# ZhuoyangLiu2005/MLA

Measured on AMD Instinct MI355X. Metric: training samples/sec + step-time, MLA-Llama2-7B bf16, higher is better.
Workload: dtype bf16; 1 GPU; BASELINE.json configs[1]: MLA-Llama2-7B SFT, use_pointcloud+use_contrastive, 672x672(+mask) image + 1024 points + 32 text tokens, per-GPU batch 8 x 4 diffusion repeats = 32 x 548 tokens; model=mla-llama2-7b, global_batch=8, seq_len=548, parallelism=single-gpu, activation_save_level=1, optimizer=fused AdamW + grad clip inside the timed region

## Files before the change

### include/mla_hip.h

```cpp
#ifndef MLA_HIP_H
#define MLA_HIP_H

#include <stddef.h>
#include <stdint.h>

#ifdef __cplusplus
extern "C" {
#endif

typedef struct ihipStream_t* mla_stream_t;

const char* mla_last_error(void);
int mla_query(int what);
const char* mla_gemm_source_id(void);
int mla_selftest(const void* src_1k, int* out_tr_256, void* out_glds_1k, mla_stream_t stream);
int mla_calib_mfma(const void* operands, float* out, int blocks, int iters, double* flops_per_launch, mla_stream_t stream);
int mla_dispatch_probe(int* out, int blocks, int hold_us, mla_stream_t stream);

int mla_gemm_bf16(const void* A, const void* B, void* C, const void* R, const void* bias, int M, int N, int K, int lda, int ldb,
                  int ldc, int ldr, int a_mode, int b_mode, int out_fp32, int accumulate, float alpha, int force_generic,
                  mla_stream_t stream);
int mla_gemm_bf16_ws(const void* A, const void* B, void* C, const void* R, const void* bias, int M, int N, int K, int lda, int ldb,
                     int ldc, int ldr, int a_mode, int b_mode, int out_fp32, int accumulate, float alpha, int force_generic,
                     float* workspace, size_t workspace_bytes, mla_stream_t stream);
// ... 42 lines not shown
int mla_act_fwd(const void* x, void* y, long long n, int kind, mla_stream_t stream);
int mla_act_bwd(const void* dy, const void* x, void* dx, long long n, int kind, mla_stream_t stream);

int mla_cast_f32_to_bf16(const float* x, void* y, long long n, mla_stream_t stream);
int mla_cast_bf16_to_f32(const void* x, float* y, long long n, mla_stream_t stream);
int mla_add_bf16(const void* a, const void* b, void* y, long long n, mla_stream_t stream);
int mla_gather_rows_bf16(const void* src, const long long* idx, void* out, long long rows, int H, int scatter, mla_stream_t stream);

int mla_transpose_bf16(const void* src, void* dst, long long R, int C, long long ld, long long ldt, mla_stream_t stream);
int mla_rmsnorm_apply_t(const void* x, const void* w, const float* rstd, void* dst, long long rows, int H, long long ldt,
                        mla_stream_t stream);
int mla_swiglu_fwd_t(const void* gu, void* dst, long long rows, int I, long long ldt, mla_stream_t stream);
int mla_swiglu_fwd_dual(const void* gu, void* act, void* actT, long long rows, int I, long long ldt, mla_stream_t stream);
int mla_swiglu_bwd_t(const void* dact, const void* gu, void* dgu, void* dguT, long long rows, int I, long long ldt, mla_stream_t stream);

int mla_embedding_fwd(const long long* ids, const void* table, void* out, long long tokens, int H, int vocab, mla_stream_t stream);
int mla_embedding_bwd(const long long* ids, const void* dy, float* grad, float* workspace, long long tokens, int H, int vocab,
                      mla_stream_t stream);

int mla_adamw_step(float* p, const float* g, float* m, float* v, void* p16, long long n, float lr, float beta1, float beta2,
                   float eps, float weight_decay, int step, const float* grad_scale, mla_stream_t stream);
int mla_adamw_step_groups(float* p, const float* g, float* m, float* v, void* p16, long long n, long long n_decay, float lr, float beta1,
                          float beta2, float eps, float weight_decay, int step, const float* grad_scale, mla_stream_t stream);
int mla_sumsq_f32(const float* x, long long n, float* out, int accumulate, float* workspace, size_t workspace_bytes,
                  mla_stream_t stream);
int mla_sum_partials(const float* partial, int n, float* out, int accumulate, mla_stream_t stream);
int mla_clip_coef(const float* sumsq, float max_norm, float* coef, float* norm_out, mla_stream_t stream);

int mla_q_sample(const float* x0, const float* noise, const long long* t, const float* sqrt_ac, const float* sqrt_1mac, float* out,
                 int batch, int per, int nsteps, mla_stream_t stream);

int mla_attn_fwd(const void* q, const void* k, const void* v, void* o, float* lse, const int* seqlens, int B, int S, int H,
                 int head_dim, long long ld_qkv, long long ld_o, float scale, mla_stream_t stream);
int mla_attn_fwd_g(const void* q, const void* k, const void* v, void* o, float* lse, const int* seqlens, int B, int S, int H,
                   int head_dim, long long ld_qkv, long long ld_o, float scale, int grp_start, int grp_len, const int* grp_starts,
                   mla_stream_t stream);
int mla_attn_bwd_g(const void* q, const void* k, const void* v, const void* o, const void* dout, const float* lse, const int* seqlens,
                   void* dq, void* dk, void* dv, float* delta, int B, int S, int H, int head_dim, long long ld_qkv, long long ld_o,
                   float scale, const float* rope_cos, const float* rope_sin, void* dqT, void* dkT, void* dvT, void* oT,
                   long long ldt, int* head_sync, long long head_sync_ints, int grp_start, int grp_len, const int* grp_starts,
                   int rope_per_sample, mla_stream_t stream);
long long mla_attn_bwd_sync_ints(int B, int H);
int mla_attn_bwd(const void* q, const void* k, const void* v, const void* o, const void* dout, const float* lse, const int* seqlens,
                 void* dq, void* dk, void* dv, float* delta, int B, int S, int H, int head_dim, long long ld_qkv, long long ld_o,
                 float scale, const float* rope_cos, const float* rope_sin, int* head_sync, long long head_sync_ints,
                 mla_stream_t stream);
// ... 170 lines not shown
```

### mla_amd/csrc/elementwise.hip

```cpp
#include "common.h"
#include <math.h>

namespace {


constexpr int NORM_MAXC = 4;

__global__ __launch_bounds__(256) void rmsnorm_fwd_kernel(const bf16_t* __restrict__ x, const bf16_t* __restrict__ w,
                                                          bf16_t* __restrict__ y, float* __restrict__ rstd_out,
                                                          int rows, int H, float eps) {
  __shared__ float scratch[16];
  const int row = blockIdx.x;
  const int nchunk = H >> 3;
  const bf16_t* xr = x + (size_t)row * H;
  float xv[NORM_MAXC][8];
  float ss = 0.f;
#pragma unroll
  for (int c = 0; c < NORM_MAXC; ++c) {
    const int ch = threadIdx.x + c * 256;
    if (ch < nchunk) {
      const u32x4_t v = *(const u32x4_t*)(xr + ch * 8);
      unpack8(v, xv[c]);
#pragma unroll
      for (int j = 0; j < 8; ++j) ss += xv[c][j] * xv[c][j];
// ... 660 lines not shown
      if (i >= hi) continue;
      const float decay = i < n4_decay ? decay_on : 1.f;
#pragma unroll
      for (int r = 0; r < 4; ++r) {
        float pp = p4[u][r], mm = m4[u][r], vv = v4[u][r];
        adamw_elem(pp, g4[u][r], mm, vv, gs, decay, beta1, beta2, step, isq, eps);
        p4[u][r] = pp; m4[u][r] = mm; v4[u][r] = vv;
      }
      if (NT) {
        __builtin_nontemporal_store(p4[u], p + i); __builtin_nontemporal_store(m4[u], m + i); __builtin_nontemporal_store(v4[u], v + i);
      } else {
        p[i] = p4[u]; m[i] = m4[u]; v[i] = v4[u];
      }
      if (p16) {
        u32x2_t o;
        o[0] = pack2bf(p4[u][0], p4[u][1]);
        o[1] = pack2bf(p4[u][2], p4[u][3]);
        if (NT) __builtin_nontemporal_store(o, p16 + i); else p16[i] = o;
      }
    }
  }
}

__global__ __launch_bounds__(256) void sumsq_partial_kernel(const float* __restrict__ x, float* __restrict__ partial, long long n) {
  __shared__ float scratch[16];
  float s0 = 0.f, s1 = 0.f;
  const long long n4 = n >> 2;
  const f32x4_t* x4 = (const f32x4_t*)x;
  for (long long i = (long long)blockIdx.x * 256 + threadIdx.x; i < n4; i += (long long)gridDim.x * 256) {
    const f32x4_t v = x4[i];
    s0 += v[0] * v[0] + v[1] * v[1];
    s1 += v[2] * v[2] + v[3] * v[3];
  }
  if (blockIdx.x == 0 && threadIdx.x < (n & 3)) { const float v = x[(n4 << 2) + threadIdx.x]; s0 += v * v; }
  const float s = block_sum(s0 + s1, scratch);
  if (threadIdx.x == 0) partial[blockIdx.x] = s;
}
__global__ __launch_bounds__(256) void sum_final_kernel(const float* __restrict__ partial, float* __restrict__ out, int P,
                                                        int accumulate) {
  __shared__ float scratch[16];
  float s = 0.f;
  int i0 = 0;
  if ((((uintptr_t)partial) & 15) == 0) {
    const f32x4_t* p4 = (const f32x4_t*)partial;
    const int n4 = P >> 2;
    f32x4_t a0 = {0.f, 0.f, 0.f, 0.f}, a1 = a0, a2 = a0, a3 = a0;
// ... 240 lines not shown
    else if (variant == 3) ADAMW_LAUNCH(1, false);
    else if (variant == 4) ADAMW_LAUNCH(2, false);
    else ADAMW_LAUNCH(4, true);
#undef ADAMW_LAUNCH
  }
  const long long done = n4 * 4;
  if (done < n)
    hipLaunchKernelGGL(adamw_kernel, dim3(grid_for(n - done, 8192)), dim3(256), 0, stream, p + done, g + done, m + done, v + done,
                       p16 ? (bf16_t*)p16 + done : (bf16_t*)nullptr, n - done, lr, beta1, beta2, eps, weight_decay, bc1, bc2, grad_scale,
                       n_decay > done ? n_decay - done : 0);
  MLA_LAUNCH_CHECK();
}
extern "C" int mla_adamw_step(float* p, const float* g, float* m, float* v, void* p16, long long n, float lr, float beta1,
                              float beta2, float eps, float weight_decay, int step, const float* grad_scale,
                              hipStream_t stream) {
  return adamw_impl(p, g, m, v, p16, n, n, lr, beta1, beta2, eps, weight_decay, step, grad_scale, stream);
}
extern "C" int mla_adamw_step_groups(float* p, const float* g, float* m, float* v, void* p16, long long n, long long n_decay, float lr,
                                     float beta1, float beta2, float eps, float weight_decay, int step, const float* grad_scale,
                                     hipStream_t stream) {
  return adamw_impl(p, g, m, v, p16, n, n_decay, lr, beta1, beta2, eps, weight_decay, step, grad_scale, stream);
}

extern "C" int mla_sumsq_f32(const float* x, long long n, float* out, int accumulate, float* workspace, size_t workspace_bytes,
                             hipStream_t stream) {
  MLA_CHECK_ARG(x && out && workspace && workspace_bytes >= 2048 * sizeof(float) && AL16(x), "mla_sumsq_f32: bad args");
  const int nb = grid_for(n / 4 + 1, 2048);
  hipLaunchKernelGGL(sumsq_partial_kernel, dim3(nb), dim3(256), 0, stream, x, workspace, n);
  hipLaunchKernelGGL(sum_final_kernel, dim3(1), dim3(256), 0, stream, workspace, out, nb, accumulate);
  MLA_LAUNCH_CHECK();
}
extern "C" int mla_sum_partials(const float* partial, int n, float* out, int accumulate, hipStream_t stream) {
  MLA_CHECK_ARG(partial && out && n >= 0, "mla_sum_partials: bad args");
  hipLaunchKernelGGL(sum_final_kernel, dim3(1), dim3(256), 0, stream, partial, out, n, accumulate);
  MLA_LAUNCH_CHECK();
}
extern "C" int mla_clip_coef(const float* sumsq, float max_norm, float* coef, float* norm_out, hipStream_t stream) {
  MLA_CHECK_ARG(sumsq && coef, "mla_clip_coef: bad args");
  hipLaunchKernelGGL(clip_coef_kernel, dim3(1), dim3(1), 0, stream, sumsq, max_norm, coef, norm_out);
  MLA_LAUNCH_CHECK();
}

extern "C" int mla_q_sample(const float* x0, const float* noise, const long long* t, const float* sqrt_ac,
                            const float* sqrt_1mac, float* out, int batch, int per, int nsteps, hipStream_t stream) {
  MLA_CHECK_ARG(x0 && noise && t && sqrt_ac && sqrt_1mac && out, "mla_q_sample: null pointer");
  hipLaunchKernelGGL(q_sample_kernel, dim3((batch * per + 255) / 256), dim3(256), 0, stream, x0, noise, t, sqrt_ac, sqrt_1mac,
// ... 12 lines not shown
```

### mla_amd/fsdp.py

```python
from __future__ import annotations

from typing import Callable, Dict, List, Optional, Sequence, Tuple

import torch
import torch.distributed as dist
import torch.nn as nn


class HipLocalOps:

    def __init__(self):
        from . import hip
        self.hip = hip

    def cast_to_bf16(self, src32, dst16):
        self.hip.cast_f32_to_bf16(src32, dst16)

    def adamw(self, p32, g32, m, v, p16, lr, betas, eps, wd, step, grad_scale):
        self.hip.adamw_step(p32, g32, m, v, p16, lr, betas[0], betas[1], eps, wd, step, grad_scale)

    def adamw_groups(self, p32, g32, m, v, p16, n_decay, lr, betas, eps, wd, step, grad_scale):
        self.hip.adamw_step_groups(p32, g32, m, v, p16, n_decay, lr, betas[0], betas[1], eps, wd, step, grad_scale)

    def sumsq(self, x32, out1, accumulate):
        self.hip.sumsq(x32, out1, accumulate)

    def sum_partials(self, partials, n, out1, accumulate):
        self.hip.sum_partials(partials, n, out1, accumulate)

    def clip_coef(self, sumsq1, max_norm, coef1, norm1):
        self.hip.clip_coef(sumsq1, max_norm, coef1, norm1)

    def stream(self, device):
        return torch.cuda.Stream(device=device)


class _SqArena:

    def __init__(self, n: int, device):
        self.buf = torch.zeros(n, dtype=torch.float32, device=device)
        self.used = 0

    def take(self, count: int):
        if self.used + count > self.buf.numel():
            return None
# ... 19 lines not shown
            done[k] = env[k]
    return done


def default_no_decay(n: str, p) -> bool:
    return p.ndim <= 1 or n.endswith(".bias")


def plan_flat_layout(named_params: Sequence[Tuple[str, nn.Parameter]], world: int, no_decay: Callable = default_no_decay):
    decay = [(n, p) for n, p in named_params if p.requires_grad and not no_decay(n, p)]
    nodecay = [(n, p) for n, p in named_params if p.requires_grad and no_decay(n, p)]
    frozen = [(n, p) for n, p in named_params if not p.requires_grad]
    align = 8 * world
    params: List[Tuple[str, nn.Parameter, int]] = []
    off = 0
    bounds = []
    for group in (decay, nodecay, frozen):
        for n, p in group:
            params.append((n, p, off))
            off += _round_up(p.numel(), 8)
        off = _round_up(off, align)
        bounds.append(off)
    return params, bounds[0], bounds[1], bounds[2]


def discover_units(model: nn.Module, unit_policy: Callable[[nn.Module], bool]):
    unit_mods: List[Tuple[str, nn.Module]] = []

    def walk(prefix, mod):
        for cn, child in mod.named_children():
            full = f"{prefix}.{cn}" if prefix else cn
            if unit_policy(child):
                unit_mods.append((full, child))
            else:
                walk(full, child)
    walk("", model)
    claimed = set()
    pending = []
    for name, mod in unit_mods:
        named = [(f"{name}.{n}", p) for n, p in mod.named_parameters() if id(p) not in claimed]
        claimed.update(id(p) for _, p in named)
        pending.append((name, mod, named))
    root_named = [(n, p) for n, p in model.named_parameters() if id(p) not in claimed]
    early = [x for x in pending if not hasattr(x[1], "self_attn")]
    layers = [x for x in pending if hasattr(x[1], "self_attn")]
    out = list(early)
    if root_named:
        out.append(("<root>", None, root_named))
    out.extend(layers)
    return [x for x in out if x[2]]


def plan_sharded_layout(model: nn.Module, unit_policy: Callable[[nn.Module], bool], world: int, no_decay: Callable = default_no_decay,
                        inplace_reduce: bool = True):
    units = []
    for name, mod, named in discover_units(model, unit_policy):
        params, n_decay, n_train, n_total = plan_flat_layout(named, world, no_decay)
        shard_train, shard_frozen = n_train // world, (n_total - n_train) // world
        ranges = []
        for rank in range(world):
            lo, hi = rank * shard_train, (rank + 1) * shard_train
            ranges.append([(max(a, lo) - lo, min(b, hi) - lo, max(a, lo), dec) for a, b, dec in ((0, n_decay, True), (n_decay, n_train, False))
                           if min(b, hi) > max(a, lo)])
        units.append(dict(name=name, is_layer=mod is not None and hasattr(mod, "self_attn"), params=params, n_decay=n_decay, n_train=n_train,
                          n_total=n_total, shard_train=shard_train, shard_frozen=shard_frozen, shard_ranges=ranges,
                          bytes_bf16_replica=2 * n_total, bytes_grad32=4 * n_train,
                          bytes_master=4 * (shard_train + shard_frozen), bytes_moments=8 * shard_train,
                          bytes_grad_shard=0 if (inplace_reduce or world == 1) else 4 * shard_train))
    return units


class _Arenas:

    ALIGN_BYTES = 2 << 20

    def __init__(self, sizes: Dict[str, int], device, slices: int = 0):
        dt = {"flat16": torch.bfloat16}
        pad = {k: slices * (self.ALIGN_BYTES // (2 if k == "flat16" else 4)) for k in sizes}
        self.buf = {k: torch.zeros(max(n + pad[k], 1), dtype=dt.get(k, torch.float32), device=device) for k, n in sizes.items() if n > 0}
        self.used = {k: 0 for k in self.buf}

    def has(self, kind: str) -> bool:
        return kind in self.buf

    def take(self, kind: str, n: int):
        if n == 0:
            return torch.zeros(0, dtype=torch.bfloat16 if kind == "flat16" else torch.float32, device=next(iter(self.buf.values())).device)
        gran = self.ALIGN_BYTES // self.buf[kind].element_size()
        o = (self.used[kind] + gran - 1) // gran * gran
        assert o + n <= self.buf[kind].numel(), f"arena {kind}: {o} + {n} > {self.buf[kind].numel()}"
        self.used[kind] = o + n
        return self.buf[kind][o:o + n]


class FlatUnit:

    def __init__(self, name: str, named_params: Sequence[Tuple[str, nn.Parameter]], device, world: int, rank: int, ops,
                 no_decay: Callable[[str, nn.Parameter], bool], process_group=None, sync_from_rank0: bool = True,
                 collectives: Optional[bool] = None, inplace_reduce: bool = False, arenas: Optional["_Arenas"] = None):
        self.name, self.world, self.rank, self.ops, self.device = name, world, rank, ops, device
        def take(kind, n, dtype):
            if arenas is not None and arenas.has(kind):
                return arenas.take(kind, n)
            return torch.zeros(n, dtype=dtype, device=device)
        coll = (world > 1) if collectives is None else collectives
        self.params, self.n_decay, self.n_train, self.n_total = plan_flat_layout(named_params, world, no_decay)
        self.shard_total = self.n_total // world
        self.shard_train = self.n_train // world
        self.trainable = self.n_train > 0

        full32 = torch.zeros(self.n_total, dtype=torch.float32, device=device)
        for n, p, o in self.params:
            full32[o:o + p.numel()].copy_(p.detach().reshape(-1).to(device=device, dtype=torch.float32))
        if coll and sync_from_rank0:
            dist.broadcast(full32, src=0, group=process_group)
        self.flat16 = take("flat16", self.n_total, torch.bfloat16)
        ops.cast_to_bf16(full32, self.flat16)
        nf = (self.n_total - self.n_train) // world
        if not coll and not (arenas is not None and arenas.has("master")):
            self.master_train, self.master_frozen = full32[:self.n_train], full32[self.n_train:]
        else:
            r = rank if coll else 0
# ... 9 lines not shown
            if not coll:
                self.gshard = self.grad32
            elif self.inplace_reduce:
                self.gshard = self.grad32[rank * self.shard_train:(rank + 1) * self.shard_train]
            else:
                self.gshard = take("gshard", self.shard_train, torch.float32)
            self.exp_avg = take("exp_avg", self.shard_train, torch.float32)
            self.exp_avg_sq = take("exp_avg_sq", self.shard_train, torch.float32)
        self.sq_entries: Dict[int, Tuple[int, int, int]] = {}
        self.sq_arena = None
        self._offset_of = {id(p): o for _, p, o in self.params}
        for n, p, o in self.params:
            p.data = self.flat16[o:o + p.numel()].view(p.shape)
            if p.requires_grad:
                p.main_grad = self.grad32[o:o + p.numel()].view(p.shape)
                p._mg_touched = False
                p._mg_dirty = False
                if not coll and hasattr(ops, "sum_partials"):
                    p._sq_sink = self._sq_sink
                    p._sq_invalidate = self._sq_invalidate_param
            p.grad = None
        self.gather_event = None
        self.rs_event = None

    def sq_invalidate(self, off: int, end: int) -> None:
        if not self.sq_entries:
            return
        for k in [k for k, e in self.sq_entries.items() if k < end and off < k + e[0]]:
            e = self.sq_entries.pop(k)
            self.sq_arena.buf[e[1]:e[1] + e[2]].zero_()

    def _sq_invalidate_param(self, p) -> None:
        off = self._offset_of.get(id(p))
        if off is not None:
            self.sq_invalidate(off, off + p.numel())

    def _sq_sink(self, weights, count):
        arena = self.sq_arena
        if arena is None:
            return None
        off = self._offset_of[id(weights[0])]
        end = self._offset_of[id(weights[-1])] + weights[-1].numel()
        self.sq_invalidate(off, end)
        part = arena.take(count)
        if part is None:
            return None
# ... 60 lines not shown
                if p.grad is not None:
                    raise RuntimeError(f"{self.name}: {n} received an autograd gradient after the unit's reduce-scatter was launched")
                if not p._mg_touched and any(getattr(p, "_mg_regions", {}).values()):
                    p._mg_touched = True
                if not p._mg_touched and p._mg_dirty:
                    raise RuntimeError(f"{self.name}: {n} holds a stale gradient that was reduced with this step's (untouched this step, "
                                       "but the unit's reduce-scatter fired from its backward hook)")
                if p._mg_touched:
                    p._mg_dirty = True
            return
        self.collect_autograd_grads()
        for _, p, _ in self.params:
            if p.requires_grad:
                if not p._mg_touched and any(getattr(p, "_mg_regions", {}).values()):
                    p._mg_touched = True
                if not p._mg_touched and p._mg_dirty:
                    p.main_grad.zero_()
                    p._mg_dirty = False
                elif p._mg_touched:
                    p._mg_dirty = True

    def state_bytes(self):
        n = self.flat16.numel() * 2 + (self.master_train.numel() + self.master_frozen.numel()) * 4
        if self.trainable:
            n += self.grad32.numel() * 4 + (self.exp_avg.numel() + self.exp_avg_sq.numel()) * 4
            if self.gshard is not self.grad32 and not self.inplace_reduce:
                n += self.gshard.numel() * 4
        return n


class ShardedModel:

    def __init__(self, model: nn.Module, unit_policy: Callable[[nn.Module], bool], device, ops=None,
                 process_group=None, no_decay: Optional[Callable[[str, nn.Parameter], bool]] = None,
                 inplace_reduce: Optional[bool] = None):
        self.model, self.device = model, device
        self.pg = process_group
        import os
        self.world = dist.get_world_size(process_group) if dist.is_available() and dist.is_initialized() else 1
        self.rank = dist.get_rank(process_group) if self.world > 1 else 0
        self.coll = self.world > 1 or (os.environ.get("MLA_FORCE_COLLECTIVES") == "1" and dist.is_available() and dist.is_initialized())
        self.ops = ops if ops is not None else HipLocalOps()
        if inplace_reduce is None and os.environ.get("MLA_FSDP_INPLACE_RS") == "0":
            inplace_reduce = False
        self.inplace_reduce = bool(self.coll and (dist.get_backend(process_group) == "nccl" if inplace_reduce is None else inplace_reduce))
        self.sum_shards = bool(self.inplace_reduce or (self.coll and dist.get_backend(process_group) == "nccl"))
        self.grad_div = float(self.world) if self.sum_shards else 1.0
        no_decay = no_decay or default_no_decay
        self.units: List[FlatUnit] = []
        self.unit_of_module: Dict[int, FlatUnit] = {}
        found = discover_units(model, unit_policy)
        self._arenas = None
        kinds = [k for k in os.environ.get("MLA_FSDP_ARENAS", "master,exp_avg,exp_avg_sq").split(",") if k and k != "0"]
        if kinds:
            sizes = dict(flat16=0, grad32=0, master=0, exp_avg=0, exp_avg_sq=0, gshard=0)
            for name, mod, named in found:
                _, n_decay, n_train, n_total = plan_flat_layout(named, self.world, no_decay)
                w = self.world if self.coll else 1
                sizes["flat16"] += n_total
                sizes["grad32"] += n_train
                sizes["master"] += n_total // w
                sizes["exp_avg"] += n_train // self.world
                sizes["exp_avg_sq"] += n_train // self.world
                if self.coll and not self.inplace_reduce:
                    sizes["gshard"] += n_train // self.world
            self._arenas = _Arenas({k: v for k, v in sizes.items() if k in kinds}, device, slices=2 * len(found))
        for name, mod, named in found:
            self._add_unit(name, mod, named, no_decay)
        for b in model.buffers():
            b.data = b.data.to(device)
        self.step_count = 0
        self.defer_reduce = False
        self._sumsq = torch.zeros(1, dtype=torch.float32, device=device)
        self._sq_arena = _SqArena(1 << 20, device) if (not self.coll and hasattr(self.ops, "sum_partials") and
                                                       self.device.type == "cuda") else None
        for u in self.units:
            u.sq_arena = self._sq_arena
        self._coef = torch.ones(1, dtype=torch.float32, device=device)
        self._norm = torch.zeros(1, dtype=torch.float32, device=device)
        self.on_gpu = self.device.type == "cuda"
        if self.on_gpu:
            assert torch.cuda.current_device() == (self.device.index or 0), \
                f"torch.cuda.set_device({self.device}) must be called before sharding a model onto it"
        self.comm_stream = self.ops.stream(device) if self.coll else None
        self.wait_profile = None
        if self.on_gpu and self.comm_stream is not None:
            for u in self.units:
                mod = getattr(u, "module", None)
                if mod is not None:
                    mod.register_forward_pre_hook(lambda m, inp, uu=u: self.wait_unit(uu))
                    if hasattr(mod, "_gather_wait"):
                        mod._gather_wait = (lambda uu=u: self.wait_unit(uu))
                else:
                    owned = {id(p) for _, p, _ in u.params}
                    for m in model.modules():
                        if any(id(p) in owned for p in m.parameters(recurse=False)):
                            m.register_forward_pre_hook(lambda mm, inp, uu=u: self.wait_unit(uu))
        for u in self.units:
            mod = getattr(u, "module", None)
            if mod is not None and hasattr(mod, "_grad_hook") and u.trainable and self.coll:
                mod._grad_hook = (lambda uu=u: self._launch_reduce_scatter(uu))

    def _add_unit(self, name, mod, named, no_decay):
        if not named:
            return
        u = FlatUnit(name, named, self.device, self.world, self.rank, self.ops, no_decay, self.pg, collectives=self.coll,
                     inplace_reduce=self.inplace_reduce, arenas=self._arenas)
        u.module = mod
        self.units.append(u)

    def _launch_reduce_scatter(self, u: FlatUnit):
        if not self.coll or not u.trainable or u.rs_event is not None or self.defer_reduce:
            return
        u.zero_stale_and_lock()
        cur = torch.cuda.current_stream(self.device) if self.device.type == "cuda" else None
        if cur is not None:
            ev = torch.cuda.Event()
            ev.record(cur)
            with torch.cuda.stream(self.comm_stream):
                self.comm_stream.wait_event(ev)
                self._reduce_scatter(u)
                u.rs_event = torch.cuda.Event()
                u.rs_event.record(self.comm_stream)
        else:
            self._reduce_scatter(u)
            u.rs_event = True

    def _reduce_scatter(self, u: FlatUnit):
        backend = dist.get_backend(self.pg)
        if backend == "nccl":
            dist.reduce_scatter_tensor(u.gshard, u.grad32, op=dist.ReduceOp.SUM, group=self.pg)
        else:
            dist.all_reduce(u.grad32, op=dist.ReduceOp.SUM, group=self.pg)
            if not u.inplace_reduce:
                u.gshard.copy_(u.grad32[self.rank * u.shard_train:(self.rank + 1) * u.shard_train] / self.world)

    def _all_gather(self, u: FlatUnit):
        region = u.flat16[:u.n_train]
        shard = region[self.rank * u.shard_train:(self.rank + 1) * u.shard_train]
        if dist.get_backend(self.pg) == "nccl":
            dist.all_gather_into_tensor(region, shard, group=self.pg)
        else:
            parts = [torch.empty_like(shard) for _ in range(self.world)]
            dist.all_gather(parts, shard.clone(), group=self.pg)
            region.copy_(torch.cat(parts))

    def _timed_wait(self, kind: str, event) -> None:
        cur = torch.cuda.current_stream(self.device)
        prof = self.wait_profile
        if prof is None:
            cur.wait_event(event)
            return
        e0, e1 = torch.cuda.Event(enable_timing=True), torch.cuda.Event(enable_timing=True)
        e0.record(cur)
        cur.wait_event(event)
        e1.record(cur)
        prof.append((kind, e0, e1))

    def wait_profile_ms(self) -> Dict[str, float]:
        out: Dict[str, float] = {}
# ... 67 lines not shown
            first = False
        if self.coll:
            dist.all_reduce(self._sumsq, op=dist.ReduceOp.SUM, group=self.pg)
        if self.grad_div != 1.0:
            self._sumsq.mul_(1.0 / (self.grad_div * self.grad_div))
        self.ops.clip_coef(self._sumsq, float(max_norm) if max_norm is not None else 3.0e38, self._coef, self._norm)
        if self.grad_div != 1.0:
            self._coef.mul_(1.0 / self.grad_div)
        return self._norm

    def optimizer_step(self, lr: float, betas=(0.9, 0.999), eps: float = 1e-8, weight_decay: float = 0.0):
        self.step_count += 1

        for u in self.units:
            if not u.trainable:
                continue
            ranges = u._shard_ranges()
            if hasattr(self.ops, "adamw_groups") and ranges and ranges[0][0] == 0 and \
                    all(ranges[i][1] == ranges[i + 1][0] and ranges[i][2] + (ranges[i][1] - ranges[i][0]) == ranges[i + 1][2]
                        for i in range(len(ranges) - 1)):
                n_local = ranges[-1][1]
                n_dec = sum(le - ls for ls, le, _, dec in ranges if dec)
                g0 = ranges[0][2]
                self.ops.adamw_groups(u.master_train[:n_local], u.gshard[:n_local], u.exp_avg[:n_local], u.exp_avg_sq[:n_local],
                                      u.flat16[g0:g0 + n_local], n_dec, lr, betas, eps, weight_decay, self.step_count, self._coef)
            else:
                for ls, le, g0, decayed in ranges:
                    self.ops.adamw(u.master_train[ls:le], u.gshard[ls:le], u.exp_avg[ls:le], u.exp_avg_sq[ls:le],
                                   u.flat16[g0:g0 + (le - ls)], lr, betas, eps, weight_decay if decayed else 0.0, self.step_count,
                                   self._coef)
            if self.coll:
                if self.on_gpu:
                    ev = torch.cuda.Event()
                    ev.record(torch.cuda.current_stream(self.device))
                    with torch.cuda.stream(self.comm_stream):
                        self.comm_stream.wait_event(ev)
                        self._all_gather(u)
                        u.gather_event = torch.cuda.Event()
                        u.gather_event.record(self.comm_stream)
                else:
                    self._all_gather(u)

    def iter_full_state_fp32(self, to_cpu_on_rank0: bool = False):
        if self.on_gpu:
            self.wait_all()
        for u in self.units:
# ... 30 lines not shown
```

### mla_amd/hip.py

```python
from __future__ import annotations

import ctypes
import os
from ctypes import c_float, c_int, c_longlong, c_size_t, c_void_p
from typing import NamedTuple, Optional

import torch

_LIB_PATH = os.environ.get("MLA_HIP_LIB") or os.path.join(os.path.dirname(os.path.abspath(__file__)), "libmla_hip.so")
_lib = None

ACT_GELU_ERF, ACT_GELU_TANH, ACT_RELU, ACT_SILU = 0, 1, 2, 3

SPLITK = os.environ.get("MLA_GEMM_SPLITK", "1") != "0"
SPLITK_WS_BYTES = int(os.environ.get("MLA_GEMM_SPLITK_WS_MB", "64")) << 20

GEMM_PROFILE = None

_SIGNATURES = {
    "mla_query": [c_int],
    "mla_selftest": [c_void_p, c_void_p, c_void_p, c_void_p],
    "mla_dispatch_probe": [c_void_p, c_int, c_int, c_void_p],
    "mla_calib_mfma": [c_void_p, c_void_p, c_int, c_int, c_void_p, c_void_p],
    "mla_gemv_bf16": [c_void_p, c_longlong, c_void_p, c_longlong, c_void_p, c_longlong, c_longlong, c_int, c_void_p, c_longlong, c_int, c_int,
# ... 75 lines not shown
    "mla_gemm_gateup_swiglu_rs": [c_void_p, c_void_p, c_void_p, c_void_p, c_void_p, c_int, c_int, c_int, c_int, c_int, c_longlong,
                                  c_void_p, c_int, c_float, c_void_p, c_void_p],
    "mla_rmsnorm_bwd_blocks": [c_int],
    "mla_timm_rmsnorm_fwd": [c_void_p, c_void_p, c_void_p, c_void_p, c_void_p, c_int, c_int, c_float, c_void_p],
    "mla_timm_rmsnorm_bwd": [c_void_p, c_void_p, c_void_p, c_void_p, c_void_p, c_void_p, c_void_p, c_int, c_int, c_int, c_void_p,
                             c_size_t, c_void_p],
    "mla_rmsnorm_bwd": [c_void_p, c_void_p, c_void_p, c_void_p, c_void_p, c_void_p, c_void_p, c_int, c_int, c_int, c_void_p,
                        c_size_t, c_void_p],
    "mla_colsum_blocks": [c_int],
    "mla_colsum_bf16": [c_void_p, c_void_p, c_int, c_int, c_int, c_int, c_void_p, c_size_t, c_void_p],
    "mla_layernorm_fwd": [c_void_p, c_void_p, c_void_p, c_void_p, c_int, c_int, c_float, c_void_p],
    "mla_rope_inplace": [c_void_p, c_void_p, c_void_p, c_longlong, c_int, c_int, c_int, c_int, c_int, c_int, c_int, c_void_p],
    "mla_swiglu_fwd": [c_void_p, c_void_p, c_longlong, c_int, c_void_p],
    "mla_swiglu_bwd": [c_void_p, c_void_p, c_void_p, c_void_p, c_longlong, c_int, c_void_p],
    "mla_act_fwd": [c_void_p, c_void_p, c_longlong, c_int, c_void_p],
    "mla_act_bwd": [c_void_p, c_void_p, c_void_p, c_longlong, c_int, c_void_p],
    "mla_cast_f32_to_bf16": [c_void_p, c_void_p, c_longlong, c_void_p],
    "mla_cast_bf16_to_f32": [c_void_p, c_void_p, c_longlong, c_void_p],
    "mla_add_bf16": [c_void_p, c_void_p, c_void_p, c_longlong, c_void_p],
    "mla_embedding_fwd": [c_void_p, c_void_p, c_void_p, c_longlong, c_int, c_int, c_void_p],
    "mla_embedding_bwd": [c_void_p, c_void_p, c_void_p, c_void_p, c_longlong, c_int, c_int, c_void_p],
    "mla_adamw_step_groups": [c_void_p, c_void_p, c_void_p, c_void_p, c_void_p, c_longlong, c_longlong, c_float, c_float, c_float, c_float,
                              c_float, c_int, c_void_p, c_void_p],
    "mla_adamw_step": [c_void_p, c_void_p, c_void_p, c_void_p, c_void_p, c_longlong, c_float, c_float, c_float, c_float,
                       c_float, c_int, c_void_p, c_void_p],
    "mla_sumsq_f32": [c_void_p, c_longlong, c_void_p, c_int, c_void_p, c_size_t, c_void_p],
    "mla_clip_coef": [c_void_p, c_float, c_void_p, c_void_p, c_void_p],
    "mla_q_sample": [c_void_p, c_void_p, c_void_p, c_void_p, c_void_p, c_void_p, c_int, c_int, c_int, c_void_p],
    "mla_attn_fwd": [c_void_p, c_void_p, c_void_p, c_void_p, c_void_p, c_void_p, c_int, c_int, c_int, c_int, c_longlong,
                     c_longlong, c_float, c_void_p],
    "mla_attn_bwd": [c_void_p, c_void_p, c_void_p, c_void_p, c_void_p, c_void_p, c_void_p, c_void_p, c_void_p, c_void_p,
                     c_void_p, c_int, c_int, c_int, c_int, c_longlong, c_longlong, c_float, c_void_p, c_void_p, c_void_p, c_longlong,
                     c_void_p],
    "mla_attn_bwd_t": [c_void_p, c_void_p, c_void_p, c_void_p, c_void_p, c_void_p, c_void_p, c_void_p, c_void_p, c_void_p,
                       c_void_p, c_int, c_int, c_int, c_int, c_longlong, c_longlong, c_float, c_void_p, c_void_p,
                       c_void_p, c_void_p, c_void_p, c_void_p, c_longlong, c_void_p, c_longlong, c_void_p],
    "mla_attn_bwd_sync_ints": [c_int, c_int],
    "mla_attn_fwd_g": [c_void_p, c_void_p, c_void_p, c_void_p, c_void_p, c_void_p, c_int, c_int, c_int, c_int, c_longlong,
                       c_longlong, c_float, c_int, c_int, c_void_p, c_void_p],
    "mla_attn_bwd_g": [c_void_p, c_void_p, c_void_p, c_void_p, c_void_p, c_void_p, c_void_p, c_void_p, c_void_p, c_void_p,
                       c_void_p, c_int, c_int, c_int, c_int, c_longlong, c_longlong, c_float, c_void_p, c_void_p,
                       c_void_p, c_void_p, c_void_p, c_void_p, c_longlong, c_void_p, c_longlong, c_int, c_int, c_void_p, c_int, c_void_p],
    "mla_attn_bwd_ws_bytes": [c_int, c_int, c_int],
    "mla_attn_bwd_ws": [c_void_p, c_void_p, c_void_p, c_void_p, c_void_p, c_void_p, c_void_p, c_void_p, c_void_p, c_void_p,
                        c_void_p, c_int, c_int, c_int, c_int, c_longlong, c_longlong, c_float, c_void_p, c_void_p,
                        c_void_p, c_void_p, c_void_p, c_void_p, c_longlong, c_void_p, c_longlong, c_void_p],
# ... 458 lines not shown
def embedding_fwd(ids, table):
    tokens = ids.numel()
    vocab, H = table.shape
    out = torch.empty((tokens, H), dtype=torch.bfloat16, device=table.device)
    call("mla_embedding_fwd", _p(ids), _p(table), _p(out), tokens, H, vocab)
    return out


def embedding_bwd(ids, dy2d, grad_f32):
    vocab, H = grad_f32.shape
    tokens = ids.numel()
    ws = torch.empty((tokens // 64, H), dtype=torch.float32, device=grad_f32.device) if tokens >= 64 else None
    call("mla_embedding_bwd", _p(ids), _p(dy2d), _p(grad_f32), _p(ws), tokens, H, vocab)


def adamw_step(p32, g32, m, v, p16, lr, beta1, beta2, eps, wd, step, grad_scale=None):
    call("mla_adamw_step", _p(p32), _p(g32), _p(m), _p(v), _p(p16), p32.numel(), float(lr), float(beta1), float(beta2),
         float(eps), float(wd), int(step), _p(grad_scale))


def adamw_step_groups(p32, g32, m, v, p16, n_decay, lr, beta1, beta2, eps, wd, step, grad_scale=None):
    call("mla_adamw_step_groups", _p(p32), _p(g32), _p(m), _p(v), _p(p16), p32.numel(), int(n_decay), float(lr), float(beta1), float(beta2),
         float(eps), float(wd), int(step), _p(grad_scale))


def sumsq(x32, out1, accumulate):
    ws = workspace(8192, x32.device)
    call("mla_sumsq_f32", _p(x32), x32.numel(), _p(out1), 1 if accumulate else 0, _p(ws), ws.numel())


def clip_coef(sumsq1, max_norm, coef1, norm1=None):
    call("mla_clip_coef", _p(sumsq1), float(max_norm), _p(coef1), _p(norm1))


def q_sample(x0, noise, t, sqrt_ac, sqrt_1mac):
    out = torch.empty_like(x0)
    batch = x0.shape[0]
    call("mla_q_sample", _p(x0), _p(noise), _p(t), _p(sqrt_ac), _p(sqrt_1mac), _p(out), batch, x0.numel() // batch,
         sqrt_ac.numel())
    return out


def _group_args(groups, B):
    start = groups[0]
    if torch.is_tensor(start):
        _req(start, torch.int32, "attention group starts")
# ... 1007 lines not shown
```

### mla_amd/ops.py

```python
from __future__ import annotations

import math
import threading
import os
from collections import namedtuple
from dataclasses import dataclass
from typing import List, Optional, Sequence

import torch

from . import hip

BF16 = torch.bfloat16


def cat_view(tensors: Sequence[torch.Tensor]) -> Optional[torch.Tensor]:
    if len(tensors) == 1:
        return tensors[0] if tensors[0].is_contiguous() else None
    t0 = tensors[0]
    K = t0.shape[1]
    ptr = t0.data_ptr()
    total = 0
    for t in tensors:
        if t.dim() != 2 or t.shape[1] != K or not t.is_contiguous() or t.data_ptr() != ptr or t.dtype != t0.dtype:
# ... 161 lines not shown
    x2 = _as2d(x)
    T, Tp = x2.shape[0], _pad_tokens(x2.shape[0])
    return x2 if Tp == T else torch.cat([x2, x2.new_zeros(Tp - T, x2.shape[1])], 0)


def _cut_rows(x2, B, S):
    return x2[:B * S].view(B, S, x2.shape[1])


def _project(x2, weights, out=None):
    if out is None:
        out = torch.empty((x2.shape[0], sum(w.shape[0] for w in weights)), dtype=BF16, device=x2.device)
    wcat = cat_view(weights)
    if wcat is not None:
        return hip.gemm(x2, wcat, out=out)
    off = 0
    for w in weights:
        n = w.shape[0]
        hip.gemm(x2, w, out=out[:, off:off + n])
        off += n
    return out


def _transposed(weights):
    wcat = cat_view(weights)
    return hip.transpose(wcat if wcat is not None else torch.cat(list(weights), 0))


def _dgrad_rows(dy, weights):
    wcat = cat_view(weights)
    if wcat is not None:
        return hip.gemm(dy, wcat, b_mode=1)
    dx, off = None, 0
    for w in weights:
        n = w.shape[0]
        dx = hip.gemm(dy[:, off:off + n].contiguous(), w, b_mode=1, residual=dx)
        off += n
    return dx


def _rmsnorm_bwd(dy, x2, w, rstd, dres, want_w):
    dx = []

    def run(dw_out, acc):
        dx.append(hip.rmsnorm_bwd(dy, x2, w, rstd, dres=dres, dw_out=dw_out, dw_accumulate=acc))

    dw = deliver_vec_grad(w, run) if want_w else run(None, False)
    return dx[0], dw
# ... 1090 lines not shown
```

Baseline: 13.88 samples/s.

## Fuse AdamW update with writing transposed bf16 weight copies for backward dgrad

Adds a tiled AdamW kernel that, besides updating master weights and moments and writing the bf16 replica, writes a transposed bf16 copy of each per-layer dgrad weight group (qkv, o, gate/up, down) through shared memory. The FSDP layer keeps these transposed copies in a new arena and registers them, so that `_transposed` in ops returns the cached copy instead of launching a transpose kernel on every backward pass. This targets the repeated per-step weight-transpose traffic. In exchange it costs extra memory for a second bf16 copy of the weights and adds a scattered transposed write to the optimizer step. The copies are invalidated on all-gather.

```diff
diff --git a/include/mla_hip.h b/include/mla_hip.h
--- a/include/mla_hip.h
+++ b/include/mla_hip.h
@@ -88,6 +88,10 @@
                    float eps, float weight_decay, int step, const float* grad_scale, mla_stream_t stream);
 int mla_adamw_step_groups(float* p, const float* g, float* m, float* v, void* p16, long long n, long long n_decay, float lr, float beta1,
                           float beta2, float eps, float weight_decay, int step, const float* grad_scale, mla_stream_t stream);
+int mla_adamw_step_groups_t(float* p, const float* g, float* m, float* v, void* p16, void* p16_t, long long n, long long n_decay,
+                            const long long* mat_off, const int* mat_rows, const int* mat_cols, const long long* mat_toff, int n_mats,
+                            float lr, float beta1, float beta2, float eps, float weight_decay, int step, const float* grad_scale,
+                            mla_stream_t stream);
 int mla_sumsq_f32(const float* x, long long n, float* out, int accumulate, float* workspace, size_t workspace_bytes,
                   mla_stream_t stream);
 int mla_sum_partials(const float* partial, int n, float* out, int accumulate, mla_stream_t stream);
diff --git a/mla_amd/csrc/elementwise.hip b/mla_amd/csrc/elementwise.hip
--- a/mla_amd/csrc/elementwise.hip
+++ b/mla_amd/csrc/elementwise.hip
@@ -706,6 +706,95 @@
   }
 }
 
+constexpr int ADAMW_T_MAX = 8;
+struct AdamwMats {
+  long long off[ADAMW_T_MAX];
+  long long toff[ADAMW_T_MAX];
+  int rows[ADAMW_T_MAX], cols[ADAMW_T_MAX];
+  int lgw[ADAMW_T_MAX];
+  int strip_end[ADAMW_T_MAX];
+  long long gap_lo[ADAMW_T_MAX + 1];
+  long long gap_end[ADAMW_T_MAX + 1];
+  long long gap_total;
+  int n_mats, n_gaps, n_strips;
+};
+template <bool NT_T>
+__global__ __launch_bounds__(256) void adamw_tiles_kernel(float* __restrict__ p, const float* __restrict__ g, float* __restrict__ m,
+                                                          float* __restrict__ v, bf16_t* __restrict__ p16, bf16_t* __restrict__ p16_t,
+                                                          AdamwMats mats, int strip_blocks, long long n_decay, float lr, float beta1,
+                                                          float beta2, float eps, float wd, float bc1, float bc2,
+                                                          const float* __restrict__ grad_scale) {
+  __shared__ unsigned short t[256][66];
+  const float gs = grad_scale ? *grad_scale : 1.f;
+  const float step = lr / bc1, isq = 1.f / sqrtf(bc2), decay_on = 1.f - lr * wd;
+  const int tid = threadIdx.x;
+  if ((int)blockIdx.x >= strip_blocks) {
+    const long long gap_total = mats.gap_total;
+    const long long stride = (long long)(gridDim.x - strip_blocks) * 256;
+    for (long long j = (long long)(blockIdx.x - strip_blocks) * 256 + tid; j < gap_total; j += stride) {
+      long long i = mats.gap_lo[0] + j;
+#pragma unroll
+      for (int k = 1; k <= ADAMW_T_MAX; ++k)
+        if (k < mats.n_gaps && j >= mats.gap_end[k - 1]) i = mats.gap_lo[k] + (j - mats.gap_end[k - 1]);
+      float pp = p[i], mm = m[i], vv = v[i];
+      adamw_elem(pp, g[i], mm, vv, gs, i < n_decay ? 1.f - lr * wd : 1.f, beta1, beta2, step, isq, eps);
+      p[i] = pp; m[i] = mm; v[i] = vv;
+      p16[i] = f2bf(pp);
+    }
+    return;
+  }
+  for (int strip = blockIdx.x; strip < mats.n_strips; strip += strip_blocks) {
+    long long off = mats.off[0], toff = mats.toff[0];
+    int rows = mats.rows[0], cols = mats.cols[0], lgw = mats.lgw[0], local = strip;
+#pragma unroll
+    for (int d = 1; d < ADAMW_T_MAX; ++d)
+      if (d < mats.n_mats && strip >= mats.strip_end[d - 1]) {
+        off = mats.off[d]; toff = mats.toff[d]; rows = mats.rows[d]; cols = mats.cols[d]; lgw = mats.lgw[d];
+        local = strip - mats.strip_end[d - 1];
+      }
+    const int scn = cols >> (6 + lgw);
+    const int r0 = (local / scn) << 6, c0 = (local % scn) << (6 + lgw);
+    const int rr = tid >> (4 + lgw), cc = (tid & ((16 << lgw) - 1)) * 4, rpp = 16 >> lgw;
+    for (int h = 0; h < (1 << lgw); ++h) {
+      f32x4_t g4[4], p4[4], m4[4], v4[4];
+      long long idx[4];
+#pragma unroll
+      for (int u = 0; u < 4; ++u) {
+        idx[u] = off + (long long)(r0 + (h * 4 + u) * rpp + rr) * cols + c0 + cc;
+        g4[u] = __builtin_nontemporal_load((const f32x4_t*)(g + idx[u])); p4[u] = __builtin_nontemporal_load((const f32x4_t*)(p + idx[u]));
+        m4[u] = __builtin_nontemporal_load((const f32x4_t*)(m + idx[u])); v4[u] = __builtin_nontemporal_load((const f32x4_t*)(v + idx[u]));
+      }
+#pragma unroll
+      for (int u = 0; u < 4; ++u) {
+#pragma unroll
+        for (int r = 0; r < 4; ++r) {
+          float pp = p4[u][r], mm = m4[u][r], vv = v4[u][r];
+          adamw_elem(pp, g4[u][r], mm, vv, gs, idx[u] + r < n_decay ? decay_on : 1.f, beta1, beta2, step, isq, eps);
+          p4[u][r] = pp; m4[u][r] = mm; v4[u][r] = vv;
+        }
+        __builtin_nontemporal_store(p4[u], (f32x4_t*)(p + idx[u])); __builtin_nontemporal_store(m4[u], (f32x4_t*)(m + idx[u]));
+        __builtin_nontemporal_store(v4[u], (f32x4_t*)(v + idx[u]));
+        u32x2_t o;
+        o[0] = pack2bf(p4[u][0], p4[u][1]);
+        o[1] = pack2bf(p4[u][2], p4[u][3]);
+        __builtin_nontemporal_store(o, (u32x2_t*)(p16 + idx[u]));
+        const int row = (h * 4 + u) * rpp + rr;
+        t[cc][row] = (unsigned short)(o[0] & 0xffffu); t[cc + 1][row] = (unsigned short)(o[0] >> 16);
+        t[cc + 2][row] = (unsigned short)(o[1] & 0xffffu); t[cc + 3][row] = (unsigned short)(o[1] >> 16);
+      }
+    }
+    __syncthreads();
+    for (int it = 0; it < (2 << lgw); ++it) {
+      const int oc = (tid >> 3) + it * 32, orr = (tid & 7) * 8;
+      const uint32_t* q = (const uint32_t*)&t[oc][orr];
+      const u32x4_t w = {q[0], q[1], q[2], q[3]};
+      u32x4_t* dst = (u32x4_t*)(p16_t + toff + (long long)(c0 + oc) * rows + r0 + orr);
+      if (NT_T) __builtin_nontemporal_store(w, dst); else *dst = w;
+    }
+    __syncthreads();
+  }
+}
+
 __global__ __launch_bounds__(256) void sumsq_partial_kernel(const float* __restrict__ x, float* __restrict__ partial, long long n) {
   __shared__ float scratch[16];
   float s0 = 0.f, s1 = 0.f;
@@ -992,6 +1081,46 @@
   return adamw_impl(p, g, m, v, p16, n, n_decay, lr, beta1, beta2, eps, weight_decay, step, grad_scale, stream);
 }
 
+extern "C" int mla_adamw_step_groups_t(float* p, const float* g, float* m, float* v, void* p16, void* p16_t, long long n,
+                                       long long n_decay, const long long* mat_off, const int* mat_rows, const int* mat_cols,
+                                       const long long* mat_toff, int n_mats, float lr, float beta1, float beta2, float eps,
+                                       float weight_decay, int step, const float* grad_scale, hipStream_t stream) {
+  MLA_CHECK_ARG(p && g && m && v && p16 && p16_t && n >= 0 && step >= 1 && n_decay >= 0 && n_decay <= n,
+                "mla_adamw_step_groups_t: bad args");
+  MLA_CHECK_ARG(n_mats >= 1 && n_mats <= ADAMW_T_MAX && mat_off && mat_rows && mat_cols && mat_toff,
+                "mla_adamw_step_groups_t: 1 to %d matrix groups", ADAMW_T_MAX);
+  MLA_CHECK_ARG(AL16(p) && AL16(g) && AL16(m) && AL16(v) && AL16(p16) && AL16(p16_t), "mla_adamw_step_groups_t: 16-B alignment");
+  static const int max_lgw = getenv("MLA_ADAMW_T_STRIP") ? atoi(getenv("MLA_ADAMW_T_STRIP")) : 2;
+  AdamwMats mats = {};
+  long long pos = 0, strips = 0, gap_total = 0;
+  for (int d = 0; d < n_mats; ++d) {
+    const long long r = mat_rows[d], c = mat_cols[d], o = mat_off[d], to = mat_toff[d];
+    MLA_CHECK_ARG(r > 0 && c > 0 && r % 64 == 0 && c % 64 == 0, "mla_adamw_step_groups_t: group %d is [%lld, %lld], need multiples of 64", d, r, c);
+    MLA_CHECK_ARG(o >= pos && o % 8 == 0 && o + r * c <= n, "mla_adamw_step_groups_t: group %d out of order, overlapping, misaligned or past n", d);
+    MLA_CHECK_ARG(to >= 0 && to % 8 == 0, "mla_adamw_step_groups_t: group %d: bad transposed offset", d);
+    for (int e = 0; e < d; ++e)
+      MLA_CHECK_ARG(to >= mat_toff[e] + (long long)mat_rows[e] * mat_cols[e] || to + r * c <= mat_toff[e],
+                    "mla_adamw_step_groups_t: transposed images of groups %d and %d overlap", e, d);
+    if (o > pos) { mats.gap_lo[mats.n_gaps] = pos; gap_total += o - pos; mats.gap_end[mats.n_gaps++] = gap_total; }
+    pos = o + r * c;
+    const int lgw = (c % 256 == 0 && max_lgw >= 2) ? 2 : ((c % 128 == 0 && max_lgw >= 1) ? 1 : 0);
+    strips += (r / 64) * (c >> (6 + lgw));
+    MLA_CHECK_ARG(strips < (1LL << 31), "mla_adamw_step_groups_t: too many tiles");
+    mats.off[d] = o; mats.toff[d] = to; mats.rows[d] = (int)r; mats.cols[d] = (int)c; mats.lgw[d] = lgw; mats.strip_end[d] = (int)strips;
+  }
+  if (pos < n) { mats.gap_lo[mats.n_gaps] = pos; gap_total += n - pos; mats.gap_end[mats.n_gaps++] = gap_total; }
+  mats.n_mats = n_mats; mats.n_strips = (int)strips; mats.gap_total = gap_total;
+  const float bc1 = (float)(1.0 - pow((double)beta1, step)), bc2 = (float)(1.0 - pow((double)beta2, step));
+  static const int plain_t = getenv("MLA_ADAMW_T_PLAIN") ? atoi(getenv("MLA_ADAMW_T_PLAIN")) : 0;
+  const int strip_blocks = (int)(strips < adamw_grid_cap() ? strips : adamw_grid_cap());
+  const int gap_blocks = gap_total ? grid_for(gap_total, 1024) : 0;
+#define ADAMW_T_LAUNCH(NT) hipLaunchKernelGGL((adamw_tiles_kernel<NT>), dim3(strip_blocks + gap_blocks), dim3(256), 0, stream, p, g, m, v, \
+                       (bf16_t*)p16, (bf16_t*)p16_t, mats, strip_blocks, n_decay, lr, beta1, beta2, eps, weight_decay, bc1, bc2, grad_scale)
+  if (plain_t) ADAMW_T_LAUNCH(false); else ADAMW_T_LAUNCH(true);
+#undef ADAMW_T_LAUNCH
+  MLA_LAUNCH_CHECK();
+}
+
 extern "C" int mla_sumsq_f32(const float* x, long long n, float* out, int accumulate, float* workspace, size_t workspace_bytes,
                              hipStream_t stream) {
   MLA_CHECK_ARG(x && out && workspace && workspace_bytes >= 2048 * sizeof(float) && AL16(x), "mla_sumsq_f32: bad args");
diff --git a/mla_amd/fsdp.py b/mla_amd/fsdp.py
--- a/mla_amd/fsdp.py
+++ b/mla_amd/fsdp.py
@@ -21,6 +21,15 @@
 
     def adamw_groups(self, p32, g32, m, v, p16, n_decay, lr, betas, eps, wd, step, grad_scale):
         self.hip.adamw_step_groups(p32, g32, m, v, p16, n_decay, lr, betas[0], betas[1], eps, wd, step, grad_scale)
+
+    def mat_groups(self, groups):
+        return self.hip.mat_groups(groups)
+
+    def adamw_groups_t(self, p32, g32, m, v, p16, p16_t, n_decay, mats, lr, betas, eps, wd, step, grad_scale):
+        self.hip.adamw_step_groups_t(p32, g32, m, v, p16, p16_t, n_decay, mats, lr, betas[0], betas[1], eps, wd, step, grad_scale)
+
+    def transpose_into(self, src2d, dst2d):
+        self.hip.transpose(src2d, out=dst2d)
 
     def sumsq(self, x32, out1, accumulate):
         self.hip.sumsq(x32, out1, accumulate)
@@ -86,6 +95,48 @@
         off = _round_up(off, align)
         bounds.append(off)
     return params, bounds[0], bounds[1], bounds[2]
+
+
+LAYER_DGRAD_GROUPS = ((".self_attn.q_proj.weight", ".self_attn.k_proj.weight", ".self_attn.v_proj.weight"), (".self_attn.o_proj.weight",),
+                      (".mlp.gate_proj.weight", ".mlp.up_proj.weight"), (".mlp.down_proj.weight",))
+WT_TILE = 64
+WT_CACHE_STATE_BUDGET = 144 << 30
+
+
+WT_CACHE_DEFAULT = "1"
+
+
+def wt_cache_enabled() -> bool:
+    import os
+    return os.environ.get("MLA_WT_CACHE", WT_CACHE_DEFAULT) != "0"
+
+
+def wt_cache_fits(state_bytes: int, copy_bytes: int) -> bool:
+    return copy_bytes > 0 and state_bytes + copy_bytes <= WT_CACHE_STATE_BUDGET
+
+
+def plan_transposed_groups(params, n_decay: int, tile: int = WT_TILE):
+    out, toff = [], 0
+    for group in LAYER_DGRAD_GROUPS:
+        members = []
+        for suffix in group:
+            hit = [(p, o) for n, p, o in params if n.endswith(suffix)]
+            if len(hit) != 1:
+                return None
+            members.append(hit[0])
+        p0, o0 = members[0]
+        rows, end = 0, o0
+        for p, o in members:
+            if not p.requires_grad or p.ndim != 2 or p.shape[1] != p0.shape[1] or o != end:
+                return None
+            rows, end = rows + p.shape[0], o + p.numel()
+        cols = p0.shape[1]
+        if rows % tile or cols % tile or end > n_decay:
+            return None
+        out.append((o0, rows, cols, toff))
+        toff += rows * cols
+    out.sort()
+    return out
 
 
 def discover_units(model: nn.Module, unit_policy: Callable[[nn.Module], bool]):
@@ -116,8 +167,9 @@
 
 
 def plan_sharded_layout(model: nn.Module, unit_policy: Callable[[nn.Module], bool], world: int, no_decay: Callable = default_no_decay,
-                        inplace_reduce: bool = True):
+                        inplace_reduce: bool = True, wt_cache: Optional[bool] = None):
     units = []
+    wt_cache = wt_cache_enabled() if wt_cache is None else wt_cache
     for name, mod, named in discover_units(model, unit_policy):
         params, n_decay, n_train, n_total = plan_flat_layout(named, world, no_decay)
         shard_train, shard_frozen = n_train // world, (n_total - n_train) // world
@@ -126,21 +178,27 @@
             lo, hi = rank * shard_train, (rank + 1) * shard_train
             ranges.append([(max(a, lo) - lo, min(b, hi) - lo, max(a, lo), dec) for a, b, dec in ((0, n_decay, True), (n_decay, n_train, False))
                            if min(b, hi) > max(a, lo)])
+        t_groups = plan_transposed_groups(params, n_decay) if (wt_cache and world == 1) else None
         units.append(dict(name=name, is_layer=mod is not None and hasattr(mod, "self_attn"), params=params, n_decay=n_decay, n_train=n_train,
-                          n_total=n_total, shard_train=shard_train, shard_frozen=shard_frozen, shard_ranges=ranges,
+                          n_total=n_total, t_groups=t_groups, bytes_bf16_transposed=2 * sum(r * c for _, r, c, _ in (t_groups or [])), shard_train=shard_train, shard_frozen=shard_frozen, shard_ranges=ranges,
                           bytes_bf16_replica=2 * n_total, bytes_grad32=4 * n_train,
                           bytes_master=4 * (shard_train + shard_frozen), bytes_moments=8 * shard_train,
                           bytes_grad_shard=0 if (inplace_reduce or world == 1) else 4 * shard_train))
+    state = sum(u[k] for u in units for k in ("bytes_bf16_replica", "bytes_grad32", "bytes_master", "bytes_moments", "bytes_grad_shard"))
+    if not wt_cache_fits(state, sum(u["bytes_bf16_transposed"] for u in units)):
+        for u in units:
+            u["t_groups"], u["bytes_bf16_transposed"] = None, 0
     return units
 
 
 class _Arenas:
 
+    BF16_KINDS = ("flat16", "flat16_t")
     ALIGN_BYTES = 2 << 20
 
     def __init__(self, sizes: Dict[str, int], device, slices: int = 0):
-        dt = {"flat16": torch.bfloat16}
-        pad = {k: slices * (self.ALIGN_BYTES // (2 if k == "flat16" else 4)) for k in sizes}
+        dt = {k: torch.bfloat16 for k in self.BF16_KINDS}
+        pad = {k: slices * (self.ALIGN_BYTES // (2 if k in self.BF16_KINDS else 4)) for k in sizes}
         self.buf = {k: torch.zeros(max(n + pad[k], 1), dtype=dt.get(k, torch.float32), device=device) for k, n in sizes.items() if n > 0}
         self.used = {k: 0 for k in self.buf}
 
@@ -149,7 +207,7 @@
 
     def take(self, kind: str, n: int):
         if n == 0:
-            return torch.zeros(0, dtype=torch.bfloat16 if kind == "flat16" else torch.float32, device=next(iter(self.buf.values())).device)
+            return torch.zeros(0, dtype=torch.bfloat16 if kind in self.BF16_KINDS else torch.float32, device=next(iter(self.buf.values())).device)
         gran = self.ALIGN_BYTES // self.buf[kind].element_size()
         o = (self.used[kind] + gran - 1) // gran * gran
         assert o + n <= self.buf[kind].numel(), f"arena {kind}: {o} + {n} > {self.buf[kind].numel()}"
@@ -161,7 +219,8 @@
 
     def __init__(self, name: str, named_params: Sequence[Tuple[str, nn.Parameter]], device, world: int, rank: int, ops,
                  no_decay: Callable[[str, nn.Parameter], bool], process_group=None, sync_from_rank0: bool = True,
-                 collectives: Optional[bool] = None, inplace_reduce: bool = False, arenas: Optional["_Arenas"] = None):
+                 collectives: Optional[bool] = None, inplace_reduce: bool = False, arenas: Optional["_Arenas"] = None,
+                 wt_cache: bool = False):
         self.name, self.world, self.rank, self.ops, self.device = name, world, rank, ops, device
         def take(kind, n, dtype):
             if arenas is not None and arenas.has(kind):
@@ -217,6 +276,24 @@
             p.grad = None
         self.gather_event = None
         self.rs_event = None
+        self.t_groups = plan_transposed_groups(self.params, self.n_decay) if (wt_cache and not coll and self.trainable) else None
+        self.flat16_t, self.t_views, self.t_mats, self.t_valid = None, [], None, False
+        if self.t_groups:
+            self.flat16_t = take("flat16_t", sum(r * c for _, r, c, _ in self.t_groups), torch.bfloat16)
+            self.t_mats = ops.mat_groups(self.t_groups)
+            for o, r, c, to in self.t_groups:
+                self.t_views.append((self.flat16[o:o + r * c].view(r, c), self.flat16_t[to:to + r * c].view(c, r)))
+
+    def refresh_transposed(self) -> None:
+        for src, dst in self.t_views:
+            self.ops.transpose_into(src, dst)
+        self.t_valid = bool(self.t_views)
+
+    def invalidate_transposed(self) -> None:
+        self.t_valid = False
+
+    def transposed_view(self, i: int):
+        return self.t_views[i][1] if self.t_valid else None
 
     def sq_invalidate(self, off: int, end: int) -> None:
         if not self.sq_entries:
@@ -323,6 +400,8 @@
 
     def state_bytes(self):
         n = self.flat16.numel() * 2 + (self.master_train.numel() + self.master_frozen.numel()) * 4
+        if self.flat16_t is not None:
+            n += self.flat16_t.numel() * 2
         if self.trainable:
             n += self.grad32.numel() * 4 + (self.exp_avg.numel() + self.exp_avg_sq.numel()) * 4
             if self.gshard is not self.grad32 and not self.inplace_reduce:
@@ -352,13 +431,21 @@
         self.unit_of_module: Dict[int, FlatUnit] = {}
         found = discover_units(model, unit_policy)
         self._arenas = None
-        kinds = [k for k in os.environ.get("MLA_FSDP_ARENAS", "master,exp_avg,exp_avg_sq").split(",") if k and k != "0"]
+        self.wt_cache = bool(wt_cache_enabled() and not self.coll and self.world == 1 and
+                             hasattr(self.ops, "adamw_groups_t") and torch.device(device).type == "cuda")
+        if self.wt_cache:
+            plans = [plan_flat_layout(named, 1, no_decay) for _, _, named in found]
+            self.wt_cache = wt_cache_fits(sum(6 * n_total + 12 * n_train for _, _, n_train, n_total in plans),
+                                          sum(2 * r * c for pp, n_decay, _, _ in plans for _, r, c, _ in (plan_transposed_groups(pp, n_decay) or [])))
+        kinds = [k for k in os.environ.get("MLA_FSDP_ARENAS", "master,exp_avg,exp_avg_sq,flat16_t").split(",") if k and k != "0"]
         if kinds:
-            sizes = dict(flat16=0, grad32=0, master=0, exp_avg=0, exp_avg_sq=0, gshard=0)
+            sizes = dict(flat16=0, flat16_t=0, grad32=0, master=0, exp_avg=0, exp_avg_sq=0, gshard=0)
             for name, mod, named in found:
-                _, n_decay, n_train, n_total = plan_flat_layout(named, self.world, no_decay)
+                params, n_decay, n_train, n_total = plan_flat_layout(named, self.world, no_decay)
                 w = self.world if self.coll else 1
                 sizes["flat16"] += n_total
+                if self.wt_cache:
+                    sizes["flat16_t"] += sum(r * c for _, r, c, _ in (plan_transposed_groups(params, n_decay) or []))
                 sizes["grad32"] += n_train
                 sizes["master"] += n_total // w
                 sizes["exp_avg"] += n_train // self.world
@@ -368,6 +455,12 @@
             self._arenas = _Arenas({k: v for k, v in sizes.items() if k in kinds}, device, slices=2 * len(found))
         for name, mod, named in found:
             self._add_unit(name, mod, named, no_decay)
+        if self.wt_cache:
+            from . import ops as _ops
+            for u in self.units:
+                if u.t_views:
+                    u.refresh_transposed()
+                    _ops.register_transposed(u)
         for b in model.buffers():
             b.data = b.data.to(device)
         self.step_count = 0
@@ -406,7 +499,7 @@
         if not named:
             return
         u = FlatUnit(name, named, self.device, self.world, self.rank, self.ops, no_decay, self.pg, collectives=self.coll,
-                     inplace_reduce=self.inplace_reduce, arenas=self._arenas)
+                     inplace_reduce=self.inplace_reduce, arenas=self._arenas, wt_cache=self.wt_cache)
         u.module = mod
         self.units.append(u)
 
@@ -437,6 +530,7 @@
                 u.gshard.copy_(u.grad32[self.rank * u.shard_train:(self.rank + 1) * u.shard_train] / self.world)
 
     def _all_gather(self, u: FlatUnit):
+        u.invalidate_transposed()
         region = u.flat16[:u.n_train]
         shard = region[self.rank * u.shard_train:(self.rank + 1) * u.shard_train]
         if dist.get_backend(self.pg) == "nccl":
@@ -550,6 +644,11 @@
                 n_local = ranges[-1][1]
                 n_dec = sum(le - ls for ls, le, _, dec in ranges if dec)
                 g0 = ranges[0][2]
+                if u.t_mats is not None and g0 == 0 and n_local == u.n_train:
+                    self.ops.adamw_groups_t(u.master_train, u.gshard, u.exp_avg, u.exp_avg_sq, u.flat16[:u.n_train], u.flat16_t, n_dec,
+                                            u.t_mats, lr, betas, eps, weight_decay, self.step_count, self._coef)
+                    u.t_valid = True
+                    continue
                 self.ops.adamw_groups(u.master_train[:n_local], u.gshard[:n_local], u.exp_avg[:n_local], u.exp_avg_sq[:n_local],
                                       u.flat16[g0:g0 + n_local], n_dec, lr, betas, eps, weight_decay, self.step_count, self._coef)
             else:
diff --git a/mla_amd/hip.py b/mla_amd/hip.py
--- a/mla_amd/hip.py
+++ b/mla_amd/hip.py
@@ -121,6 +121,8 @@
     "mla_embedding_bwd": [c_void_p, c_void_p, c_void_p, c_void_p, c_longlong, c_int, c_int, c_void_p],
     "mla_adamw_step_groups": [c_void_p, c_void_p, c_void_p, c_void_p, c_void_p, c_longlong, c_longlong, c_float, c_float, c_float, c_float,
                               c_float, c_int, c_void_p, c_void_p],
+    "mla_adamw_step_groups_t": [c_void_p, c_void_p, c_void_p, c_void_p, c_void_p, c_void_p, c_longlong, c_longlong, c_void_p, c_void_p,
+                                c_void_p, c_void_p, c_int, c_float, c_float, c_float, c_float, c_float, c_int, c_void_p, c_void_p],
     "mla_adamw_step": [c_void_p, c_void_p, c_void_p, c_void_p, c_void_p, c_longlong, c_float, c_float, c_float, c_float,
                        c_float, c_int, c_void_p, c_void_p],
     "mla_sumsq_f32": [c_void_p, c_longlong, c_void_p, c_int, c_void_p, c_size_t, c_void_p],
@@ -625,6 +627,25 @@
 def adamw_step_groups(p32, g32, m, v, p16, n_decay, lr, beta1, beta2, eps, wd, step, grad_scale=None):
     call("mla_adamw_step_groups", _p(p32), _p(g32), _p(m), _p(v), _p(p16), p32.numel(), int(n_decay), float(lr), float(beta1), float(beta2),
          float(eps), float(wd), int(step), _p(grad_scale))
+
+
+class MatGroups(NamedTuple):
+    off: ctypes.Array
+    rows: ctypes.Array
+    cols: ctypes.Array
+    toff: ctypes.Array
+    count: int
+
+
+def mat_groups(groups) -> MatGroups:
+    k = len(groups)
+    return MatGroups((c_longlong * k)(*[int(g[0]) for g in groups]), (c_int * k)(*[int(g[1]) for g in groups]),
+                     (c_int * k)(*[int(g[2]) for g in groups]), (c_longlong * k)(*[int(g[3]) for g in groups]), k)
+
+
+def adamw_step_groups_t(p32, g32, m, v, p16, p16_t, n_decay, mats: MatGroups, lr, beta1, beta2, eps, wd, step, grad_scale=None):
+    call("mla_adamw_step_groups_t", _p(p32), _p(g32), _p(m), _p(v), _p(p16), _p(p16_t), p32.numel(), int(n_decay), mats.off, mats.rows,
+         mats.cols, mats.toff, mats.count, float(lr), float(beta1), float(beta2), float(eps), float(wd), int(step), _p(grad_scale))
 
 
 def sumsq(x32, out1, accumulate):
diff --git a/mla_amd/ops.py b/mla_amd/ops.py
--- a/mla_amd/ops.py
+++ b/mla_amd/ops.py
@@ -207,8 +207,29 @@
     return out
 
 
+_WT_COPIES = {}
+
+
+def register_transposed(unit) -> None:
+    import weakref
+    ref = weakref.ref(unit)
+    for i, (src, _) in enumerate(unit.t_views):
+        _WT_COPIES[(src.data_ptr(), src.shape[0], src.shape[1])] = (ref, i)
+
+
 def _transposed(weights):
     wcat = cat_view(weights)
+    if wcat is not None and _WT_COPIES:
+        key = (wcat.data_ptr(), wcat.shape[0], wcat.shape[1])
+        hit = _WT_COPIES.get(key)
+        if hit is not None:
+            unit = hit[0]()
+            if unit is None:
+                del _WT_COPIES[key]
+            else:
+                wt = unit.transposed_view(hit[1])
+                if wt is not None:
+                    return wt
     return hip.transpose(wcat if wcat is not None else torch.cat(list(weights), 0))
 
 
```

Measured after the change: 13.92 samples/s, median of 6. Within noise of the previous version (+0.3%).
